# AdamYuan/Adypt

Measured on AMD Instinct MI355X. Metric: Mrays/sec (primary+secondary) Sponza 1920x1080 8-bounce; % HBM-read roofline, higher is better.
Workload: dtype f32; 1 GPU; sponza-like procedural stand-in (stand-in), 248964 triangles, 1920x1080, full wavefront path trace, maxBounce 8, tmpLifetime 16, 1 spp per step; one radiance gather per timed region; frames_in_flight=32, rays_warmup=62962782, comm=none, comm_ranks=0, devices=device 0, bounces_in_one_launch=True, rehearsal=False

## Files before the change

### adypt_amd/csrc/device/context.hpp

```cpp
#pragma once
#include "traverse.hpp"
#include "path.hpp"
#include "frame_plan.hpp"
#include "tunables.hpp"
#include "resources.hpp"
#include "../../../include/adypt_hip.h"

#include <string>
#include <vector>

using namespace adypt;

namespace {

constexpr int kMaxBounce = 32;
constexpr int kMaxFramesInFlight = 128;
constexpr int kRollMaxPixels = 1 << 22;
constexpr int kDefaultPipes = 1;

struct FrameCounters {
	uint32_t count[kMaxBounce + 1][kNumSegments * kCursorStride];
	uint32_t cursor[kMaxBounce + 1][kNumSegments * kCursorStride];
	uint32_t sh_count[kMaxBounce + 1][kNumSegments * kCursorStride];
	uint32_t sh_cursor[kMaxBounce + 1][kNumSegments * kCursorStride];
};

struct EventPair { Event a, b; int kind = 0; };

struct Pipe {
	Stream stream;
	Event done;
	FrameCounters *counters = nullptr;
	uint2 *spill = nullptr;
};

struct QueueWindow { size_t offset; uint32_t seg_cap; };

struct Queues {
	Buffer<float4> o[2], d[2], col[2], hit;
	Buffer<float4> done;
	Buffer<float4> sh_o, sh_d, sh_col, sh_hit;
	Buffer<RayStats> ray_stats;
};

}

struct adypt_ctx {
	int device = 0;
	std::string error;
	Tunables tun;

	static constexpr int kSobolSlots = 4;
	Pipe pipes[kMaxPipes];
	hipStream_t stream = nullptr;
	Event fork_ev;
// ... 101 lines not shown
```

### adypt_amd/csrc/device/frame_schedule.hpp

```cpp
#pragma once
#include "context.hpp"
#include "../../../include/adypt_host.h"

namespace {

struct PassArgs { SceneArgs sc; PixelArgs px; bool stats; };
PassArgs pass_args(const adypt_ctx *c)
{
	PassArgs a;
	fill_scene(c, &a.sc); fill_pixels(c, &a.px);
	a.stats = (c->instrumentation & 2) != 0;
	return a;
}

void launch_resolve(adypt_ctx *c, const FrameArgs &f, const PassArgs &a, int first, int count)
{
	const dim3 grid((c->n_local_px + 255) / 256), block(256);
	if(c->noise_stats) hipLaunchKernelGGL(k_resolve_noise, grid, block, 0, c->stream, f, a.sc, a.px, c->d_noise_moments.get(), first, count);
	else hipLaunchKernelGGL(k_resolve, grid, block, 0, c->stream, f, a.sc, a.px, first, count);
}

int resolve_batch_frames(adypt_ctx *c, int first, int count)
{
	if(count <= 0) return ADYPT_OK;
// ... 15 lines not shown
	return ADYPT_OK;
}

void drop_rolling(adypt_ctx *c)
{
	if(c->roll_frame[0] < 0 && c->roll_frame[1] < 0) return;
	(void)hipSetDevice(c->device);
	(void)hipStreamSynchronize(c->stream);
	for(int s = 0; s < 2; ++s) { (void)hipStreamSynchronize(c->pipes[1 + s].stream); c->roll_frame[s] = -1; }
}
inline void drop_lookahead(adypt_ctx *c) { c->ahead_count = 0; c->ahead_pos = 0; drop_rolling(c); }

int upload_sobol(adypt_ctx *c, int first, int m, float *dst)
{
	const int max_bounce = c->params.max_bounce;
	const int slot = c->sobol_next;
	c->sobol_next = (slot + 1) % adypt_ctx::kSobolSlots;
	HIP_TRY(c, hipEventSynchronize(c->sobol_done[slot]));
	std::vector<float> pts((size_t)m * 2 * max_bounce);
	int r = adypt_sobol_points(2 * max_bounce, first, m, pts.data());
	if(r != ADYPT_OK) return fail(c, r, adypt_host_last_error());
	float *padded = c->h_sobol[slot];
	memset(padded, 0, (size_t)m * 64 * sizeof(float));
	for(int k = 0; k < m; ++k) memcpy(&padded[(size_t)k * 64], &pts[(size_t)k * 2 * max_bounce], sizeof(float) * 2 * (size_t)max_bounce);
	HIP_TRY(c, hipMemcpyAsync(dst, padded, (size_t)m * 64 * sizeof(float), hipMemcpyHostToDevice, c->stream));
	HIP_TRY(c, hipEventRecord(c->sobol_done[slot], c->stream));
	return ADYPT_OK;
}

void launch_shade_first(adypt_ctx *c, hipStream_t stream, int k, const QueueWindow &win, const FrameArgs &f, const PassArgs &a)
{
	FrameCounters *ctr = c->pipes[k].counters;
	hipEvent_t stop = begin_timing(c, 1, stream);
	QueueArgs q = queue_args(c, win, 0, ctr->count[0], ctr->count[1], f.n_frames);
	audit_before(c, q, stream, k);
	hipLaunchKernelGGL(k_shade_first, dim3((unsigned)(c->n_local_px / kShadeThreads)), dim3(kShadeThreads), 0, stream, f, a.sc, q, a.px, a.stats ? 1 : 0);
	audit_after(c, q, stream, k);
	end_timing(stop, stream);
}

void roll_frame_args(const adypt_ctx *c, const PassPlan &p, int frame, int s, FrameArgs *f)
{
	fill_frame(c, f);
	f->spp = frame; f->n_frames = 1; f->frame_first = 0; f->frame_stride = 1; f->batched = 1;
	f->sun_query = p.sun_query;
	f->sobol = c->d_sobol + (size_t)s * 64;
	f->done = c->q.done + (size_t)s * (size_t)std::max(c->n_local_px, 64);
}

int roll_launch(adypt_ctx *c, const PassPlan &p, const PassArgs &a, int frame, int s)
{
	const Pipe &pipe = c->pipes[1 + s];
	const QueueWindow win = pipe_window(c, s, 2);
	FrameArgs f;
	roll_frame_args(c, p, frame, s, &f);
	int r = upload_sobol(c, frame, 1, c->d_sobol + (size_t)s * 64);
	if(r != ADYPT_OK) return r;
	if(frame % std::max(1, c->params.tmp_lifetime) == 0)
	{
		FrameArgs fc = f;
		fc.frame_stride = std::max(1, c->params.tmp_lifetime);
// ... 215 lines not shown
```

### adypt_amd/csrc/device/path.hpp

```cpp
#pragma once
#include "traverse.hpp"
#include "path_limits.hpp"

namespace adypt {

#ifndef ADYPT_PATH_SLOTS
#define ADYPT_PATH_SLOTS 352
#endif
constexpr int kPathSlots = ADYPT_PATH_SLOTS;
static_assert(kPathSlots >= kTraceThreads && kPathSlots <= 2 * kTraceThreads && kPathSlots % 32 == 0, "k_path: 256 <= slots <= 512");
constexpr int kTabFields = 10;
constexpr int kRareCap = 96;
static_assert(kRareCap >= 64 && kRareCap % 8 == 0 && kRareCap + 64 <= kTraceThreads, "k_path: the deferred ring holds a round's worth (rare_min <= 64), keeps PathCtl 16-byte aligned behind it, and leaves the to-shade ring a full batch when every path waits");
constexpr int kParkDwords = 8;
constexpr uint32_t kRingMiss = 0x8000u;
constexpr uint32_t kPwIdMask = (1u << kPwBounceShift) - 1u;
enum { T_PW = 0, T_DX, T_DY, T_DZ, T_CX, T_CY, T_CZ, T_OX, T_OY, T_OZ };

struct PathCtl {
	uint32_t n_shade, n_trace, live, busy;
	uint32_t h_shade, h_trace, rays, shaded;
	uint32_t lock, init_have, h_rare, pad[5];
};

// ... 276 lines not shown
					F3 dir = f3(0, 0, 1), color = f3(0, 0, 0), origin = f3(0, 0, 0), ret = f3(0, 0, 0), ret_in = f3(0, 0, 0);
					int32_t tri_idx = -1;
					float tu = 0.0f, tv = 0.0f;
					if(have)
					{
						pw = tab[T_PW * kPathSlots + sslot];
						dir = f3(__uint_as_float(tab[T_DX * kPathSlots + sslot]), __uint_as_float(tab[T_DY * kPathSlots + sslot]), __uint_as_float(tab[T_DZ * kPathSlots + sslot]));
						color = f3(__uint_as_float(tab[T_CX * kPathSlots + sslot]), __uint_as_float(tab[T_CY * kPathSlots + sslot]), __uint_as_float(tab[T_CZ * kPathSlots + sslot]));
						if(!miss) { tri_idx = (int32_t)tab[T_OX * kPathSlots + sslot]; tu = __uint_as_float(tab[T_OY * kPathSlots + sslot]); tv = __uint_as_float(tab[T_OZ * kPathSlots + sslot]); }
					}
					const int b = (int)((pw >> kPwBounceShift) & 31u);
					const int pi = (int)(pw & kPwIdMask);
					bool parked = (pw & kPathParked) != 0u;
					const bool last = b + 1 >= f.max_bounce;
					const bool query_back = SUN && (uint32_t)b == kPwShadow, query_next = SUN && f.sun_query != 0 && !query_back && have && tri_idx == -1;
					const int frame = (int)((uint32_t)pi / (uint32_t)f.n_local_px);
					const int L = pi - frame * f.n_local_px;
					TriCore tc;
#pragma unroll
					for(int i = 0; i < 20; ++i) asm volatile("" : "=v"(tc.v[i]));
					if(have && tri_idx != -1 && !query_back)
					{
						if(a.tri_remap) tri_idx = a.tri_remap[tri_idx];
						tc = load_tri_core(sc, tri_idx);
					}
					const bool sure = have && !query_next && (tri_idx == -1 || last);
					const uint32_t n_sure = (uint32_t)__popcll(__ballot(sure));
					const bool early = n_sure != 0u && !((seg_done >> home) & 1u);
					uint32_t rel;
					asm volatile("" : "=v"(rel));
					{
// ... 14 lines not shown
						sob_x = sp2.x; sob_y = sp2.y;
					}
					if(may_defer)
					{
						const bool rare = have && tri_idx != -1 && !last && __float_as_uint(tc.v[19]) != 0u;
						const unsigned long long rm = __ballot(rare);
						if(rm != 0ull && (uint32_t)__popcll(rm) <= a.defer_max)
						{
							const uint32_t room = (uint32_t)kRareCap - n_r, rr = lane_rank(rm);
							const bool defer = rare && rr < room;
							if(defer) to_rare[ring_r(h_r + n_r + rr)] = (uint16_t)sslot;
							n_r += min((uint32_t)__popcll(rm), room);
							have = have && !defer;
						}
					}

					bool alive = have, shaded = false, bad_mat = false;
					if(have)
					{
						if(parked) ret = f3(r4.x, r4.y, r4.z);
						ret_in = ret;
						if(query_next)
						{
							dir = f3(f.sun_query_dir[0], f.sun_query_dir[1], f.sun_query_dir[2]);
							origin = f3(__uint_as_float(tab[T_OX * kPathSlots + sslot]), __uint_as_float(tab[T_OY * kPathSlots + sslot]), __uint_as_float(tab[T_OZ * kPathSlots + sslot]));
						}
						else if(tri_idx == -1)
						{
							ret = fma3(color, f3(f.sun[0], f.sun[1], f.sun[2]), ret);
							alive = false;
						}
						else if(query_back) alive = false;
						else
						{
							const SurfaceInfo si = fetch_info(f, sc, tc, tri_idx, tu, tv);
							origin = si.origin;
							if(si.bad_mat) { alive = false; bad_mat = true; }
							else
							{
								shaded = true;
								const RngPoint rng{unorm8_to_float(shift16 & 0xffu), unorm8_to_float(shift16 >> 8), sob_x, sob_y};
								alive = respond(f, si, rng, b, dir, color, ret);
							}
						}
						if(!alive)
							f.done[pi] = make_float4(gl_min(ret.x, f.clamp), gl_min(ret.y, f.clamp), gl_min(ret.z, f.clamp), 1.0f);
					}
					wave_bad += (uint32_t)__popcll(__ballot(bad_mat));
					if(count_stats) wave_shaded += (uint32_t)__popcll(__ballot(shaded));
					if(alive)
					{
						if(__float_as_uint(ret.x) != __float_as_uint(ret_in.x) || __float_as_uint(ret.y) != __float_as_uint(ret_in.y) ||
						   __float_as_uint(ret.z) != __float_as_uint(ret_in.z))
						{
							f.done[pi] = make_float4(ret.x, ret.y, ret.z, 0.0f);
							parked = true;
// ... 120 lines not shown
```

### adypt_amd/csrc/device/scene_upload.hpp

```cpp
#pragma once
#include "context.hpp"
#include "../../../include/adypt_host.h"

#include <cstring>

namespace {

constexpr long kRefTrianglesAutoMaxMB = 1l << 20;

int upload_woop(adypt_ctx *c, const adypt_scene_desc *d)
{
	std::vector<float> woop;
	const float *wp = d->woop;
	if(!wp) { woop.resize((size_t)d->n_refs * 12); adypt_woop_matrices(d->triangles, d->tri_indices, d->n_refs, woop.data()); wp = woop.data(); }
	return upload(c, &c->d_woop, wp, (size_t)d->n_refs * 12);
}

int upload_triangles(adypt_ctx *c, const adypt_scene_desc *d)
{
	std::vector<float> packed((size_t)d->n_tris * kTriFloat4 * 4, 0.0f);
	const uint8_t *src = (const uint8_t *)d->triangles;
	for(int64_t i = 0; i < d->n_tris; ++i)
	{
		float *o = packed.data() + (size_t)i * kTriFloat4 * 4;
// ... 25 lines not shown
		if(matid < 0 || matid >= d->n_mats) continue;
		memcpy(&dtex, mat + (size_t)matid * 64, 4); memcpy(&illum, mat + (size_t)matid * 64 + 48, 4); memcpy(&shininess, mat + (size_t)matid * 64 + 52, 4);
		cls[(size_t)i] = (uint8_t)material_class(illum, shininess, d->n_textures != 0 && dtex >= 0 && dtex < d->n_textures);
	}
	return upload(c, &c->d_tri_class, cls.data(), cls.size());
}

int upload_textures_and_materials(adypt_ctx *c, const adypt_scene_desc *d)
{
	std::vector<uint32_t> texels;
	std::vector<int32_t> desc;
	for(int t = 0; t < d->n_textures; ++t)
	{
		const adypt_texture &tx = d->textures[t];
		if(tx.width <= 0 || tx.height <= 0 || !tx.rgb) return fail(c, ADYPT_E_INVALID, "adypt_create: bad texture " + std::to_string(t));
		desc.push_back((int32_t)texels.size()); desc.push_back(tx.width); desc.push_back(tx.height); desc.push_back(0);
		const size_t base = texels.size(), row = (size_t)tx.width + 1;
		if(base + row * (size_t)tx.height >= ((size_t)1 << 31)) return fail(c, ADYPT_E_INVALID, "adypt_create: more than 2^31 texels");
		texels.resize(base + row * (size_t)tx.height);
		for(int y = 0; y < tx.height; ++y)
		{
			uint32_t *o = texels.data() + base + row * (size_t)y;
			const uint8_t *in = tx.rgb + (size_t)y * tx.width * 3;
			for(int x = 0; x < tx.width; ++x) o[x] = (uint32_t)in[x * 3] | (uint32_t)in[x * 3 + 1] << 8 | (uint32_t)in[x * 3 + 2] << 16 | 0xff000000u;
			o[tx.width] = o[0];
		}
	}
	TRY_CREATE(upload(c, &c->d_texels, texels.data(), texels.size()));
	std::vector<uint8_t> mats((size_t)std::max<int64_t>(d->n_mats, 1) * kMatFloat4 * 16, 0);
	for(int64_t m = 0; m < d->n_mats; ++m)
	{
// ... 38 lines not shown
```

### adypt_amd/csrc/device/shade.hpp

```cpp
#pragma once
#include "canon_math.hpp"
#include "tile_layout.hpp"
#include "noise.hpp"

namespace adypt {

constexpr int kTraceThreads = 256;
constexpr int kLdsStackMax = 8;
constexpr int kNumSegments = 8;
constexpr int kCursorStride = 32;
constexpr int kShadeThreads = 256;
constexpr int kTriFloat4 = 8;
constexpr int kMatFloat4 = 5;
constexpr uint32_t kPathParked = 0x80000000u;
constexpr uint32_t kPathIdMask = 0x7fffffffu;
constexpr uint32_t kPathShadow = 0x40000000u;

struct DeviceStats {
	unsigned long long rays, nodes, tris, hits, shaded, overflows, bad_materials;
	uint32_t max_stack, pad;
	unsigned long long wave_profile[8];
	unsigned long long clock_cycles, clock_ticks;
	unsigned long long path_rays, path_nodes, path_tris, path_hits, path_shaded;
	unsigned long long audit_errors;
	uint32_t *host_overflow;
};
__device__ __forceinline__ void report_overflow(DeviceStats *st) { atomicAdd(&st->overflows, 1ull); *st->host_overflow = 1u; }

// ... 10 lines not shown
	uint32_t *cursor;
	uint2 *spill;
	DeviceStats *stats;
	uint32_t seg_cap;
	int32_t stack_size, lds_depth;
	uint32_t refill_min, chunk, bite, endgame;
	uint32_t packed;
	float tmin;
};

struct FrameArgs {
	float inv_proj[16], inv_view[16];
	float origin[3], tmin;
	float sun[3], clamp;
	const float *sobol;
	float4 *done;
	int32_t width, height;
	int32_t spp, subpixel, tmp_life, max_bounce;
	float sun_query_dir[3];
	int32_t sun_query;
	int32_t n_frames;
	int32_t frame_first, frame_stride;
	int32_t batched;
	int32_t n_local_px;
	int32_t blocks_x;
	int32_t rank, nranks;
	int32_t n_tris, n_mats, n_tex;
	int32_t deal_chunks;
};

struct SceneArgs {
	const float4 *triangles;
	const float4 *materials;
	const uint32_t *texels;
	const int32_t *local_blocks;
	const uint8_t *tri_class;
};

constexpr uint32_t kClassMiss = 0, kClassNone = 7;
// ... 167 lines not shown
	int x, y;
	if(L >= f.n_local_px || !local_pixel_xy(f, sc.local_blocks, L, &x, &y)) return;
	float4 acc = px.accum[L];
	NoiseMoments m = f.spp + first == 0 ? NoiseMoments{0.0f, 0.0f} : moments[L];
	for(int k = first; k < first + count; ++k)
	{
		const float4 r = f.done[(size_t)k * f.n_local_px + L];
		const float fs = (float)(f.spp + k), fs1 = (float)(f.spp + k + 1);
		acc = make_float4(fmaf(acc.x, fs, r.x) / fs1, fmaf(acc.y, fs, r.y) / fs1, fmaf(acc.z, fs, r.z) / fs1, 1.0f);
		m = noise_add_sample(m, f.spp + k, r.x, r.y, r.z);
	}
	px.accum[L] = acc;
	moments[L] = m;
}

__device__ __forceinline__ int pos_mod(int a, int n) { int r = a % n; return r < 0 ? r + n : r; }

struct __attribute__((packed, aligned(4))) TexelPair { uint32_t a, b; };
__device__ inline F3 sample_texture(const SceneArgs &sc, int4 d, float s, float t)
{
	const int w = d.y, h = d.z;
	const uint32_t *tx = sc.texels + d.x;
	const float uu = fmaf(s, (float)w, -0.5f), vv = fmaf(t, (float)h, -0.5f);
	float fu = floorf(uu), fv = floorf(vv);
	const float a = uu - fu, b = vv - fv;
	fu = gl_min(gl_max(fu, -1e9f), 1e9f); fv = gl_min(gl_max(fv, -1e9f), 1e9f);
	const int i0 = pos_mod((int)fu, w), j0 = pos_mod((int)fv, h);
	const int j1 = j0 + 1 == h ? 0 : j0 + 1;
	const TexelPair r0 = *(const TexelPair *)(tx + (size_t)j0 * (size_t)(w + 1) + i0), r1 = *(const TexelPair *)(tx + (size_t)j1 * (size_t)(w + 1) + i0);
	auto rgb = [](uint32_t p) { return f3(unorm8_to_float(p), unorm8_to_float(p >> 8), unorm8_to_float(p >> 16)); };
	const float w00 = (1.0f - a) * (1.0f - b), w10 = a * (1.0f - b), w01 = (1.0f - a) * b, w11 = a * b;
	F3 r = rgb(r0.a) * w00;
	r = fma3(rgb(r0.b), w10, r);
	r = fma3(rgb(r1.a), w01, r);
	r = fma3(rgb(r1.b), w11, r);
	return r;
}

struct TriCore { float v[20]; };
__device__ __forceinline__ TriCore load_tri_core(const SceneArgs &sc, int tri_idx)
{
	const float4 *p = sc.triangles + (size_t)tri_idx * kTriFloat4;
	const float4 a = p[0], b = p[1], c = p[2], d = p[3], e = p[4];
	TriCore t;
// ... 6 lines not shown
{
	F3 r = f3(a[0], a[1], a[2]) * u;
	r = fma3(f3(b[0], b[1], b[2]), v, r);
	r = fma3(f3(c[0], c[1], c[2]), w, r);
	return r;
}
__device__ __forceinline__ F3 textured_diffuse(const SceneArgs &sc, int tri_idx, int4 desc, float u, float v, float w)
{
	const float4 *p = sc.triangles + (size_t)tri_idx * kTriFloat4 + 5;
	const float4 a = p[0], b = p[1];
	const float ts = fmaf(b.x, w, fmaf(a.z, v, a.x * u));
	const float tt = fmaf(b.y, w, fmaf(a.w, v, a.y * u));
	return sample_texture(sc, desc, ts, tt);
}

struct Rng { float sx, sy; const float *sobol; };
__device__ __forceinline__ void sobol2(const Rng &r, int i, float *x, float *y)
{
	const float a = r.sobol[2 * i] + r.sx, b = r.sobol[2 * i + 1] + r.sy;
	*x = a - floorf(a); *y = b - floorf(b);
}
struct RngPoint { float sx, sy, qx, qy; };
__device__ __forceinline__ void sobol2(const RngPoint &r, int, float *x, float *y)
{
	const float a = r.qx + r.sx, b = r.qy + r.sy;
	*x = a - floorf(a); *y = b - floorf(b);
}
template <class RNG>
__device__ inline F3 sample_hemisphere(const RNG &rng, int b, float e)
{
	float rx, ry; sobol2(rng, b, &rx, &ry);
	rx *= 6.28318530718f;
	float sin_phi, cos_phi; canon_sincos(rx, &sin_phi, &cos_phi);
	const float cos_theta = canon_pow(1.0f - ry, 1.0f / (e + 1.0f));
	const float sin_theta = sqrtf(fmaf(-cos_theta, cos_theta, 1.0f));
	return normalize3(f3(sin_theta * cos_phi, sin_theta * sin_phi, cos_theta));
}
__device__ inline F3 align_direction(F3 dir, F3 target)
{
	const F3 a = fabsf(target.x) > 0.01f ? f3(0, 1, 0) : f3(1, 0, 0);
	const F3 u = normalize3(cross3(a, target));
	const F3 v = cross3(target, u);
	F3 r = u * dir.x;
	r = fma3(v, dir.y, r);
	r = fma3(target, dir.z, r);
	return r;
}

__device__ __forceinline__ void finish_path(const FrameArgs &f, const PixelArgs &px, int pi, int L, F3 ret)
{
	const F3 r = f3(gl_min(ret.x, f.clamp), gl_min(ret.y, f.clamp), gl_min(ret.z, f.clamp));
// ... 1 lines not shown
	const float4 old = px.accum[L];
	const float fs = (float)f.spp, fs1 = (float)(f.spp + 1);
	px.accum[L] = make_float4(fmaf(old.x, fs, r.x) / fs1, fmaf(old.y, fs, r.y) / fs1, fmaf(old.z, fs, r.z) / fs1, 1.0f);
}

struct SurfaceInfo { F3 origin, normal, diffuse, specular, emission; int illum0; float shininess, ior; bool bad_mat; };
__device__ __forceinline__ SurfaceInfo fetch_info(const FrameArgs &f, const SceneArgs &sc, const TriCore &tc, int tri_idx, float tu, float tv)
{
	SurfaceInfo s;
	const float *tri = tc.v;
	const int matid = __float_as_int(tri[18]);
	const float w = 1.0f - tu - tv;
	s.normal = normalize3(bary3(tri + 9, tri + 12, tri + 15, tu, tv, w));
	s.origin = bary3(tri + 0, tri + 3, tri + 6, tu, tv, w);
	s.bad_mat = matid < 0 || matid >= f.n_mats;
	s.diffuse = s.specular = s.emission = f3(0, 0, 0); s.illum0 = 0; s.shininess = 0.0f; s.ior = 1.0f;
	if(!s.bad_mat)
	{
		const float4 *mp = sc.materials + (size_t)matid * kMatFloat4;
		const float4 md = mp[0], me = mp[1], ms = mp[2], mx = mp[3], mt = mp[4];
		const int dtex = __float_as_int(md.x);
		s.illum0 = __float_as_int(mx.x); s.shininess = mx.y; s.ior = mx.w;
		const int4 tex_desc = make_int4(__float_as_int(mt.x), __float_as_int(mt.y), __float_as_int(mt.z), 0);
		if(f.n_tex != 0 && dtex != -1 && dtex >= 0 && dtex < f.n_tex) s.diffuse = textured_diffuse(sc, tri_idx, tex_desc, tu, tv, w);
		else s.diffuse = f3(md.y, md.z, md.w);
		s.specular = f3(ms.y, ms.z, ms.w);
		s.emission = f3(me.y, me.z, me.w);
	}
	return s;
}

__device__ __forceinline__ SurfaceInfo fetch_info(const FrameArgs &f, const SceneArgs &sc, int tri_idx, float tu, float tv)
{
	return fetch_info(f, sc, load_tri_core(sc, tri_idx), tri_idx, tu, tv);
}

template <class RNG>
__device__ __forceinline__ bool respond(const FrameArgs &f, const SurfaceInfo &si, const RNG &rng, int b, F3 &dir, F3 &color, F3 &ret)
// ... 74 lines not shown
	uint32_t local = chunk * kShadeThreads + threadIdx.x;
	if(sc.tri_class)
	{
		uint32_t key = kClassNone;
		if(local < n_in)
		{
			const int tri = __float_as_int(q.hit[3 * ((size_t)seg * q.seg_cap + local)]);
			key = tri < 0 || tri >= f.n_tris ? kClassMiss : (uint32_t)sc.tri_class[tri];
		}
		local = chunk * kShadeThreads + bin_by_key(key);
	}
	const uint32_t slot_in = seg * q.seg_cap + local;
	bool alive = local < n_in;
	F3 origin = f3(0, 0, 0), dir = f3(0, 0, 1), color = f3(0, 0, 0), ret = f3(0, 0, 0);
	int L = 0, pi = 0;
	const float *sobol = f.sobol;
	bool shaded = false, bad_mat = false, parked = false, escaped = false;
	F3 ret_in = f3(0, 0, 0);
	if(alive)
	{
		const float4 rd = q.ray_d[slot_in];
		const F3 h = ld3(q.hit, slot_in);
		color = ld3(q.col, slot_in);
		dir = f3(rd.x, rd.y, rd.z);
		pi = (int)(__float_as_uint(rd.w) & kPathIdMask);
		L = pi;
		if(f.batched)
		{
			const int frame = (int)((uint32_t)pi / (uint32_t)f.n_local_px);
			L = pi - frame * f.n_local_px;
			sobol += frame * 64;
		}
		parked = (__float_as_uint(rd.w) & kPathParked) != 0u;
		if(parked) { const float4 r4 = f.done[pi]; ret = f3(r4.x, r4.y, r4.z); }
		ret_in = ret;
		const int tri_idx = __float_as_int(h.x);
		const float tu = h.y, tv = h.z;
		if(store_cache) px.cache[L] = make_float4(h.x, tu, tv, 0.0f);

		if(tri_idx == -1)
		{
			if(sh.enabled) escaped = true;
			else ret = fma3(color, f3(f.sun[0], f.sun[1], f.sun[2]), ret);
			alive = false;
		}
		else
		{
			const SurfaceInfo si = fetch_info(f, sc, tri_idx, tu, tv);
			origin = si.origin;
			if(si.bad_mat) { alive = false; bad_mat = true; }
			else
			{
				shaded = true;
				const uint8_t *sh = px.shift + (size_t)L * 2;
				const Rng rng{unorm8_to_float(sh[0]), unorm8_to_float(sh[1]), sobol};
				alive = respond(f, si, rng, b, dir, color, ret);
			}
		}
		if(!alive && !escaped) finish_path(f, px, pi, L, ret);
	}
	{
		const unsigned long long mb = __ballot(bad_mat);
		if(mb && (threadIdx.x & 63) == 0) atomicAdd(&px.stats->bad_materials, (unsigned long long)__popcll(mb));
		if(count_stats)
		{
			const int n_shaded = __syncthreads_count(shaded);
			if(n_shaded && threadIdx.x == 0) atomicAdd(&px.stats->shaded, (unsigned long long)n_shaded);
		}
	}
	const uint32_t slot = append_slot(alive, q.count_out + seg * kCursorStride, seg * q.seg_cap);
// ... 23 lines not shown
}

__global__ __launch_bounds__(kShadeThreads, 7) void k_shade(FrameArgs f, SceneArgs sc, QueueArgs q, PixelArgs px, ShadowArgs sh, int b, int store_cache, int count_stats)
{
	const uint32_t seg = blockIdx.x & (kNumSegments - 1), chunk = blockIdx.x >> 3;
	const uint32_t n_in = q.count_in[seg * kCursorStride];
	if(chunk * kShadeThreads >= n_in) return;
	shade_chunk(f, sc, q, px, sh, b, store_cache, count_stats, seg, chunk, n_in);
}

__global__ __launch_bounds__(kShadeThreads, 6) void k_shade_first(FrameArgs f, SceneArgs sc, QueueArgs q, PixelArgs px, int count_stats)
{
	const uint32_t L = blockIdx.x * kShadeThreads + threadIdx.x;
	int x = 0, y = 0;
	const bool valid = L < (uint32_t)f.n_local_px && local_pixel_xy(f, sc.local_blocks, (int)L, &x, &y);
	Rng rng{0.0f, 0.0f, f.sobol};
	if(valid)
	{
		const uint8_t *sh = px.shift + (size_t)L * 2;
		rng.sx = unorm8_to_float(sh[0]); rng.sy = unorm8_to_float(sh[1]);
	}
	SurfaceInfo si;
	si.origin = si.normal = si.diffuse = si.specular = si.emission = f3(0, 0, 0); si.illum0 = 0; si.shininess = 0.0f; si.ior = 1.0f; si.bad_mat = false;
	F3 cam_dir = f3(0, 0, 1);
	bool hit = false;
	int group_now = -1;
	unsigned long long n_shaded = 0, n_bad = 0;
	for(int ordinal = 0; ordinal < f.n_frames; ++ordinal)
	{
		const int frame = f.frame_first + ordinal * f.frame_stride;
		const int group = frame_group(f, frame);
		if(group != group_now)
		{
			group_now = group;
			if(valid)
			{
// ... 5 lines not shown
				hit = tri_idx != -1;
				if(hit) si = fetch_info(f, sc, tri_idx, h.y, h.z);
			}
		}
		const int pi = frame * f.n_local_px + (int)L;
		bool alive = valid, query = false;
		F3 dir = cam_dir, color = f3(1.0f, 1.0f, 1.0f), ret = f3(0, 0, 0);
		if(valid)
		{
			if(!hit && f.sun_query) { query = true; dir = f3(f.sun_query_dir[0], f.sun_query_dir[1], f.sun_query_dir[2]); }
			else if(!hit) { ret = fma3(color, f3(f.sun[0], f.sun[1], f.sun[2]), ret); alive = false; }
			else if(si.bad_mat) { alive = false; ++n_bad; }
			else
			{
				++n_shaded;
				Rng r = rng; r.sobol = f.sobol + frame * 64;
				alive = respond(f, si, r, 0, dir, color, ret);
			}
			if(!alive) finish_path(f, px, pi, (int)L, ret);
		}
		const uint32_t seg = ((uint32_t)ordinal * gridDim.x + blockIdx.x) & (kNumSegments - 1);
		const uint32_t slot = append_slot(alive, q.count_out + seg * kCursorStride, seg * q.seg_cap);
		if(alive)
		{
			if(query) st3(q.out_o, slot, f.origin[0], f.origin[1], f.origin[2]);
			else st3(q.out_o, slot, si.origin.x, si.origin.y, si.origin.z);
			bool parked = false;
			if(__float_as_uint(ret.x) != 0u || __float_as_uint(ret.y) != 0u || __float_as_uint(ret.z) != 0u)
			{
				f.done[pi] = make_float4(ret.x, ret.y, ret.z, 0.0f);
				parked = true;
			}
// ... 37 lines not shown
__device__ __forceinline__ F3 viewer_color(const FrameArgs &f, const SceneArgs &sc, DeviceStats *stats, int tri_idx, float u, float v, int viewer_type)
{
	F3 color = f3(0, 0, 0);
	if(tri_idx == -1) return color;
	const int matid = __float_as_int(sc.triangles[(size_t)tri_idx * kTriFloat4 + 4].z);
	if(matid < 0 || matid >= f.n_mats) { atomicAdd(&stats->bad_materials, 1ull); return color; }
	const float4 *mp = sc.materials + (size_t)matid * kMatFloat4;
	const float w = 1.0f - u - v;
	if(viewer_type == 0)
	{
		const float4 md = mp[0];
		const int dtex = __float_as_int(md.x);
		if(f.n_tex != 0 && dtex != -1 && dtex >= 0 && dtex < f.n_tex)
		{
			const float4 mt = mp[4];
			color = textured_diffuse(sc, tri_idx, make_int4(__float_as_int(mt.x), __float_as_int(mt.y), __float_as_int(mt.z), 0), u, v, w);
		}
		else color = f3(md.y, md.z, md.w);
	}
	else if(viewer_type == 1) { const float4 ms = mp[2]; color = f3(ms.y, ms.z, ms.w); }
	else if(viewer_type == 2) { const float4 me = mp[1]; color = f3(me.y, me.z, me.w); }
	else if(viewer_type == 4 || viewer_type == 5)
	{
		const TriCore tc = load_tri_core(sc, tri_idx);
		const float *tri = tc.v;
		color = viewer_type == 4 ? normalize3(bary3(tri + 9, tri + 12, tri + 15, u, v, w)) : bary3(tri + 0, tri + 3, tri + 6, u, v, w);
	}
	return color;
}

__device__ __forceinline__ uint32_t unorm8(float c)
// ... 73 lines not shown
```

### adypt_amd/csrc/device/tracer.hip

```cpp
#include "context.hpp"
#include "ctx_access.hpp"
#include "../../../include/adypt_hip.h"
#include "../../../include/adypt_host.h"

#include <algorithm>
#include <atomic>
#include <cstdio>
#include <cstdlib>
#include <cstring>
#include <string>
#include <type_traits>
#include <vector>

using namespace adypt;

namespace {

thread_local std::string g_create_error;

__global__ void k_clear_counters(uint4 *p, uint32_t n16) { const uint32_t i = blockIdx.x * blockDim.x + threadIdx.x; if(i < n16) p[i] = make_uint4(0, 0, 0, 0); }

constexpr uint32_t kAuditPoison = 0xffffffffu;
__global__ void k_audit_poison(float4 *out_d, size_t n, uint32_t *seen, size_t n_seen)
{
// ... 234 lines not shown
	HIP_TRY(c, hipGetLastError());
	return ADYPT_OK;
}

void fill_frame(const adypt_ctx *c, FrameArgs *f)
{
	memset(f, 0, sizeof(*f));
	memcpy(f->inv_proj, c->inv_proj, 64); memcpy(f->inv_view, c->inv_view, 64);
	memcpy(f->origin, c->origin, 12);
	f->tmin = c->params.ray_tmin;
	memcpy(f->sun, c->params.sun, 12);
	f->clamp = c->params.clamp;
	f->width = c->width; f->height = c->height;
	f->spp = c->spp; f->subpixel = c->params.subpixel; f->tmp_life = c->params.tmp_lifetime; f->max_bounce = c->params.max_bounce;
	f->sobol = c->d_sobol; f->done = c->q.done; f->n_frames = 1; f->frame_first = 0; f->frame_stride = 1; f->batched = 0;
	f->n_local_px = c->n_local_px; f->blocks_x = c->blocks_x; f->rank = c->rank; f->nranks = c->nranks;
	f->n_tris = (int32_t)c->n_tris; f->n_mats = (int32_t)c->n_mats; f->n_tex = c->n_tex;
	f->deal_chunks = c->deal_chunks;
	memcpy(f->sun_query_dir, c->sun_dir, 12); f->sun_query = 0;
}
void fill_scene(const adypt_ctx *c, SceneArgs *s)
{
	s->triangles = (const float4 *)c->d_triangles;
	s->materials = (const float4 *)c->d_materials;
	s->texels = (const uint32_t *)c->d_texels;
	s->local_blocks = (const int32_t *)c->d_local_blocks;
	s->tri_class = (const uint8_t *)c->d_tri_class;
}
void fill_pixels(const adypt_ctx *c, PixelArgs *p)
{
	p->accum = c->d_accum; p->cache = c->d_cache; p->cache_next = c->d_cache_next; p->shift = c->d_shift; p->stats = c->d_stats;
// ... 63 lines not shown
int load_shift(adypt_ctx *c)
{
	if(c->shift_loaded && c->shift_seed_loaded == c->params.shift_seed) return ADYPT_OK;
	std::vector<uint8_t> full((size_t)c->width * c->height * 2), local((size_t)c->n_local_px * 2, 0);
	adypt_shift_bytes(c->params.shift_seed, c->width, c->height, full.data());
	for_each_local_pixel(c->local_blocks, c->width, c->height, [&](size_t L, int x, int y) {
		local[L * 2] = full[((size_t)y * c->width + x) * 2];
		local[L * 2 + 1] = full[((size_t)y * c->width + x) * 2 + 1];
	});
	HIP_TRY(c, hipStreamSynchronize(c->stream));
	if(!local.empty()) HIP_TRY(c, hipMemcpy(c->d_shift, local.data(), local.size(), hipMemcpyHostToDevice));
	c->shift_loaded = true; c->shift_seed_loaded = c->params.shift_seed;
	return ADYPT_OK;
}

int alloc_queues_raw(adypt_ctx *c, int fif)
{
	c->q = Queues{};
	const size_t npx = (size_t)std::max(c->n_local_px, 64);
	const size_t paths = npx * (size_t)fif;
	if(paths >= ((size_t)1 << 31)) return fail(c, ADYPT_E_INVALID, "frames in flight x pixels exceeds 2^31 paths");
	c->seg_cap = seg_slots_for(c, fif);
	c->capacity = (int64_t)c->seg_cap * kNumSegments;
	c->frames_in_flight = fif;
	size_t nq = (size_t)c->capacity;
	for(int n = 2; n <= kMaxPipes; ++n)
		nq = std::max(nq, (size_t)n * kNumSegments * (size_t)seg_slots_for(c, (fif + n - 1) / n));
	c->alloc_slots = nq;
	for(int i = 0; i < 2; ++i)
	{
		HIP_TRY(c, c->q.o[i].alloc(nq * sizeof(float4)));
		HIP_TRY(c, c->q.d[i].alloc(nq * sizeof(float4)));
		HIP_TRY(c, c->q.col[i].alloc(nq * sizeof(float4)));
	}
	HIP_TRY(c, c->q.hit.alloc(nq * sizeof(float4)));
	HIP_TRY(c, c->q.done.alloc(npx * (size_t)std::max(fif, 2) * sizeof(float4)));
	return ADYPT_OK;
}

int alloc_queues(adypt_ctx *c, int fif)
{
	const int previous = c->queues_ok ? c->frames_in_flight : 0;
	int r = alloc_queues_raw(c, fif);
	c->queues_ok = r == ADYPT_OK;
	if(r == ADYPT_OK) return r;
	const std::string why = c->error;
	(void)hipGetLastError();
	if(previous > 0 && previous != fif && alloc_queues_raw(c, previous) == ADYPT_OK)
	{
		c->queues_ok = true;
		c->error = why + " (kept " + std::to_string(previous) + " frames in flight)";
// ... 832 lines not shown
```

### adypt_amd/csrc/measure/k_path_blocks.py

```python
import sys
d = sys.argv[1]
import os
COUNT = os.environ.get("ADYPT_BLOCKS_COUNT", "0") != "0"
SET = os.environ.get("ADYPT_BLOCKS_SET", "trip")
SETS = {"trip": ["setup", "exchange", "shade", "trip", "A_pop", "A_choose", "A_push", "B_tri_load", "B_node_load", "C_woop", "D_slab", "E_flush"],
        "shade": ["shade", "S_parked", "S_miss", "S_surface", "S_textured", "S_glossy", "S_diffuse", "S_mirror", "S_dielectric", "S_dead", "S_alive", "S_replace"],
        "rare": ["trip", "shade", "A_pop_spill", "A_push_spill", "div_slow", "S_fetch_more", "S_early", "X_lock_spin", "exchange", "setup", "F_try", "S_defer"]}
LANES = os.environ.get("ADYPT_BLOCKS_LANES", "0") != "0"
SETS_LANES = {"trip": ["trip", "A_choose", "C_woop", "D_slab", "E_flush"], "shade": ["S_surface", "S_textured", "S_glossy", "S_diffuse", "S_dielectric"],
              "rare": ["S_miss", "S_mirror", "S_dead", "S_alive", "S_replace"],
              "wait": ["W_idle", "W_wait", "W_two", "W_three", "W_four"]}
NAMES = SETS_LANES[SET] if LANES else SETS[SET]


def edit(name, pairs):
    p = d + "/" + name
    s = open(p).read()
    for old, new in pairs:
        assert s.count(old) == 1, (name, s.count(old), old[:70])
        s = s.replace(old, new)
    open(p, "w").write(s)


def enter(n):
# ... 50 lines not shown
    ("						if(parked) r4 = f.done[pi];", "						if(parked) { " + enter("S_parked") + " r4 = f.done[pi]; " + leave("S_parked") + " }"),
    ("							ret = fma3(color, f3(f.sun[0], f.sun[1], f.sun[2]), ret); // pathtracer.glsl:130-135 (a query that came back empty: the sun is visible)\n							alive = false;",
     "							" + enter("S_miss") + "\n							ret = fma3(color, f3(f.sun[0], f.sun[1], f.sun[2]), ret); // pathtracer.glsl:130-135 (a query that came back empty: the sun is visible)\n							alive = false;\n							" + leave("S_miss")),
    ("							const SurfaceInfo si = fetch_info(f, sc, tc, tri_idx, tu, tv);", "							" + enter("S_surface") + "\n							const SurfaceInfo si = fetch_info(f, sc, tc, tri_idx, tu, tv);"),
    ("						if(rm != 0ull && (uint32_t)__popcll(rm) <= a.defer_max)\n						{", "						if(rm != 0ull && (uint32_t)__popcll(rm) <= a.defer_max)\n						{\n							" + enter("S_defer")),
    ("							have = have && !defer;\n						}", "							have = have && !defer;\n							" + leave("S_defer") + "\n						}"),
    ("								alive = respond(f, si, rng, b, dir, color, ret);\n							}\n						}", "								alive = respond(f, si, rng, b, dir, color, ret);\n							}\n							" + leave("S_surface") + "\n						}"),
    ("						if(!alive) // main()'s clamp (pathtracer.glsl:224); the running mean is k_resolve's, in frame order (a k_path pass is always batched)\n							f.done[pi] = make_float4(gl_min(ret.x, f.clamp), gl_min(ret.y, f.clamp), gl_min(ret.z, f.clamp), 1.0f);",
     "						if(!alive) { " + enter("S_dead") + "\n							f.done[pi] = make_float4(gl_min(ret.x, f.clamp), gl_min(ret.y, f.clamp), gl_min(ret.z, f.clamp), 1.0f); " + leave("S_dead") + " }"),
    ("					if(alive)\n					{\n						if(__float_as_uint(ret.x) != __float_as_uint(ret_in.x)", "					if(alive)\n					{\n						" + enter("S_alive") + "\n						if(__float_as_uint(ret.x) != __float_as_uint(ret_in.x)"),
    ("						tab[T_OX * kPathSlots + sslot] = __float_as_uint(origin.x); tab[T_OY * kPathSlots + sslot] = __float_as_uint(origin.y); tab[T_OZ * kPathSlots + sslot] = __float_as_uint(origin.z);\n					}\n					// ---------------- paths that ended",
     "						tab[T_OX * kPathSlots + sslot] = __float_as_uint(origin.x); tab[T_OY * kPathSlots + sslot] = __float_as_uint(origin.y); tab[T_OZ * kPathSlots + sslot] = __float_as_uint(origin.z);\n						" + leave("S_alive") + "\n					}\n					// ---------------- paths that ended"),
    ("					if(repl) load_path(a, idx, sslot);", "					if(repl) { " + enter("S_replace") + " load_path(a, idx, sslot); " + leave("S_replace") + " }"),
]
SHADE_HPP = [
    ("		if(f.n_tex != 0 && dtex != -1 && dtex >= 0 && dtex < f.n_tex) s.diffuse = textured_diffuse(sc, tri_idx, tex_desc, tu, tv, w);\n		else s.diffuse = f3(md.y, md.z, md.w);\n		s.specular = f3(ms.y, ms.z, ms.w);",
     "		if(f.n_tex != 0 && dtex != -1 && dtex >= 0 && dtex < f.n_tex) { " + enter("S_textured") + " s.diffuse = textured_diffuse(sc, tri_idx, tex_desc, tu, tv, w); " + leave("S_textured") + " }\n		else s.diffuse = f3(md.y, md.z, md.w);\n		s.specular = f3(ms.y, ms.z, ms.w);"),
    ("		if(e > 0.3f)\n		{\n			const F3 r = reflect3(dir, normal), shv = sample_hemisphere(rng, b, e);", "		if(e > 0.3f)\n		{\n			" + enter("S_glossy") + "\n			const F3 r = reflect3(dir, normal), shv = sample_hemisphere(rng, b, e);"),
    ("			done = true;\n		}\n		else illum = 1;", "			done = true;\n			" + leave("S_glossy") + "\n		}\n		else illum = 1;"),
    ("		if(illum == 1)\n		{\n			dir = align_direction(sample_hemisphere(rng, b, 0.0f), normal);\n			color = color * diffuse;\n		}",
     "		if(illum == 1)\n		{\n			" + enter("S_diffuse") + "\n			dir = align_direction(sample_hemisphere(rng, b, 0.0f), normal);\n			color = color * diffuse;\n			" + leave("S_diffuse") + "\n		}"),
    ("		else if(illum >= 3 && illum <= 5)\n		{\n			color = color * specular;\n			dir = reflect3(dir, normal);\n		}",
     "		else if(illum >= 3 && illum <= 5)\n		{\n			" + enter("S_mirror") + "\n			color = color * specular;\n			dir = reflect3(dir, normal);\n			" + leave("S_mirror") + "\n		}"),
    ("		else if(illum == 6 || illum == 7)\n		{\n			float eta = ior;", "		else if(illum == 6 || illum == 7)\n		{\n			" + enter("S_dielectric") + "\n			float eta = ior;"),
    ("			else dir = reflect3(dir, normal);\n		}\n	}\n	return alive;", "			else dir = reflect3(dir, normal);\n			" + leave("S_dielectric") + "\n		}\n	}\n	return alive;"),
]
edit("shade.hpp", SHADE_HPP)
pairs = SHADE_PATH + [
    ("						if(early && lane == 0) rel = atomicAdd(&a.cursor[cur], n_sure);", "						if(early && lane == 0) { " + enter("S_early") + " rel = atomicAdd(&a.cursor[cur], n_sure); " + leave("S_early") + " }"),
    ("						while(served < n_dead) // (wave-uniform) the rest: paths that ended unexpectedly, or the home segment has run out\n						{", "						while(served < n_dead) // (wave-uniform) the rest: paths that ended unexpectedly, or the home segment has run out\n						{\n							" + enter("S_fetch_more")),
# ... 24 lines not shown
```

Before: 8383 Mrays/s.

## Precompute hemisphere sample tables, pow2 texture wrap, and magic-number path-id division

```diff
diff --git a/adypt_amd/csrc/device/context.hpp b/adypt_amd/csrc/device/context.hpp
--- a/adypt_amd/csrc/device/context.hpp
+++ b/adypt_amd/csrc/device/context.hpp
@@ -14,6 +14,7 @@
 namespace {
 
 constexpr int kMaxBounce = 32;
+static_assert(kMaxBounce == kSampleTabBounces, "the sampling tables have a row per bounce");
 constexpr int kMaxFramesInFlight = 128;
 constexpr int kRollMaxPixels = 1 << 22;
 constexpr int kDefaultPipes = 1;
@@ -39,6 +40,7 @@
 struct Queues {
 	Buffer<float4> o[2], d[2], col[2], hit;
 	Buffer<float4> done;
+	Buffer<float2> phi_tab, theta_tab;
 	Buffer<float4> sh_o, sh_d, sh_col, sh_hit;
 	Buffer<RayStats> ray_stats;
 };
diff --git a/adypt_amd/csrc/device/frame_schedule.hpp b/adypt_amd/csrc/device/frame_schedule.hpp
--- a/adypt_amd/csrc/device/frame_schedule.hpp
+++ b/adypt_amd/csrc/device/frame_schedule.hpp
@@ -53,6 +53,8 @@
 int upload_sobol(adypt_ctx *c, int first, int m, float *dst)
 {
 	const int max_bounce = c->params.max_bounce;
+	const size_t row0 = (size_t)(dst - c->d_sobol.get()) / 64;
+	if((row0 + (size_t)m) * kSampleTabBounces * 256 * sizeof(float2) > c->q.phi_tab.bytes()) return fail(c, ADYPT_E_STATE, "upload_sobol: more frames than the sampling tables hold");
 	const int slot = c->sobol_next;
 	c->sobol_next = (slot + 1) % adypt_ctx::kSobolSlots;
 	HIP_TRY(c, hipEventSynchronize(c->sobol_done[slot]));
@@ -64,6 +66,9 @@
 	for(int k = 0; k < m; ++k) memcpy(&padded[(size_t)k * 64], &pts[(size_t)k * 2 * max_bounce], sizeof(float) * 2 * (size_t)max_bounce);
 	HIP_TRY(c, hipMemcpyAsync(dst, padded, (size_t)m * 64 * sizeof(float), hipMemcpyHostToDevice, c->stream));
 	HIP_TRY(c, hipEventRecord(c->sobol_done[slot], c->stream));
+	hipLaunchKernelGGL(k_sample_tables, dim3((unsigned)max_bounce, (unsigned)m), dim3(256), 0, c->stream, (const float *)dst,
+	                   c->q.phi_tab + row0 * kSampleTabBounces * 256, c->q.theta_tab + row0 * kSampleTabBounces * 256);
+	HIP_TRY(c, hipGetLastError());
 	return ADYPT_OK;
 }
 
@@ -84,6 +89,7 @@
 	f->spp = frame; f->n_frames = 1; f->frame_first = 0; f->frame_stride = 1; f->batched = 1;
 	f->sun_query = p.sun_query;
 	f->sobol = c->d_sobol + (size_t)s * 64;
+	f->phi_tab = c->q.phi_tab + (size_t)s * kSampleTabBounces * 256; f->theta_tab = c->q.theta_tab + (size_t)s * kSampleTabBounces * 256;
 	f->done = c->q.done + (size_t)s * (size_t)std::max(c->n_local_px, 64);
 }
 
diff --git a/adypt_amd/csrc/device/path.hpp b/adypt_amd/csrc/device/path.hpp
--- a/adypt_amd/csrc/device/path.hpp
+++ b/adypt_amd/csrc/device/path.hpp
@@ -314,7 +314,7 @@
 					bool parked = (pw & kPathParked) != 0u;
 					const bool last = b + 1 >= f.max_bounce;
 					const bool query_back = SUN && (uint32_t)b == kPwShadow, query_next = SUN && f.sun_query != 0 && !query_back && have && tri_idx == -1;
-					const int frame = (int)((uint32_t)pi / (uint32_t)f.n_local_px);
+					const int frame = (int)path_id_div((uint32_t)pi, f.px_div);
 					const int L = pi - frame * f.n_local_px;
 					TriCore tc;
 #pragma unroll
@@ -359,6 +359,13 @@
 							have = have && !defer;
 						}
 					}
+					float2 ph, th;
+					asm volatile("" : "=v"(ph.x), "=v"(ph.y), "=v"(th.x), "=v"(th.y));
+					if(have)
+					{
+						const uint32_t row = (uint32_t)(frame * kSampleTabBounces + b) * 256u;
+						ph = f.phi_tab[row + (shift16 & 0xffu)]; th = f.theta_tab[row + (shift16 >> 8)];
+					}
 
 					bool alive = have, shaded = false, bad_mat = false;
 					if(have)
@@ -384,7 +391,7 @@
 							else
 							{
 								shaded = true;
-								const RngPoint rng{unorm8_to_float(shift16 & 0xffu), unorm8_to_float(shift16 >> 8), sob_x, sob_y};
+								const RngPoint rng{shift16, sob_x, sob_y, ph, th};
 								alive = respond(f, si, rng, b, dir, color, ret);
 							}
 						}
diff --git a/adypt_amd/csrc/device/path_id_div.hpp b/adypt_amd/csrc/device/path_id_div.hpp
--- /dev/null
+++ b/adypt_amd/csrc/device/path_id_div.hpp
@@ -0,0 +1,34 @@
+#pragma once
+#include <cstdint>
+#include "path_limits.hpp"
+
+#ifndef ADYPT_HOST_DEVICE
+#ifdef __HIPCC__
+#define ADYPT_HOST_DEVICE __host__ __device__ __forceinline__
+#else
+#define ADYPT_HOST_DEVICE inline
+#endif
+#endif
+
+namespace adypt {
+
+struct PathIdDiv { uint32_t mul, shift; };
+
+inline PathIdDiv path_id_div_of(uint32_t d)
+{
+	uint32_t l = 0;
+	while(((uint64_t)1 << l) < d) ++l;
+	const uint64_t p = (uint64_t)1 << (kPwBounceShift + l);
+	return PathIdDiv{(uint32_t)((p + d - 1) / d), l};
+}
+
+ADYPT_HOST_DEVICE uint32_t path_id_div(uint32_t n, PathIdDiv d)
+{
+#ifdef __HIP_DEVICE_COMPILE__
+	return __umulhi(n << (32u - kPwBounceShift), d.mul) >> d.shift;
+#else
+	return (uint32_t)(((uint64_t)(n << (32u - kPwBounceShift)) * d.mul) >> 32) >> d.shift;
+#endif
+}
+
+}
diff --git a/adypt_amd/csrc/device/scene_upload.hpp b/adypt_amd/csrc/device/scene_upload.hpp
--- a/adypt_amd/csrc/device/scene_upload.hpp
+++ b/adypt_amd/csrc/device/scene_upload.hpp
@@ -63,7 +63,8 @@
 	{
 		const adypt_texture &tx = d->textures[t];
 		if(tx.width <= 0 || tx.height <= 0 || !tx.rgb) return fail(c, ADYPT_E_INVALID, "adypt_create: bad texture " + std::to_string(t));
-		desc.push_back((int32_t)texels.size()); desc.push_back(tx.width); desc.push_back(tx.height); desc.push_back(0);
+		desc.push_back((int32_t)texels.size()); desc.push_back(tx.width); desc.push_back(tx.height);
+		desc.push_back(is_pow2(tx.width) && is_pow2(tx.height) ? 1 : 0);
 		const size_t base = texels.size(), row = (size_t)tx.width + 1;
 		if(base + row * (size_t)tx.height >= ((size_t)1 << 31)) return fail(c, ADYPT_E_INVALID, "adypt_create: more than 2^31 texels");
 		texels.resize(base + row * (size_t)tx.height);
diff --git a/adypt_amd/csrc/device/shade.hpp b/adypt_amd/csrc/device/shade.hpp
--- a/adypt_amd/csrc/device/shade.hpp
+++ b/adypt_amd/csrc/device/shade.hpp
@@ -2,6 +2,8 @@
 #include "canon_math.hpp"
 #include "tile_layout.hpp"
 #include "noise.hpp"
+#include "path_id_div.hpp"
+#include "texture_wrap.hpp"
 
 namespace adypt {
 
@@ -12,6 +14,7 @@
 constexpr int kShadeThreads = 256;
 constexpr int kTriFloat4 = 8;
 constexpr int kMatFloat4 = 5;
+constexpr int kSampleTabBounces = 32;
 constexpr uint32_t kPathParked = 0x80000000u;
 constexpr uint32_t kPathIdMask = 0x7fffffffu;
 constexpr uint32_t kPathShadow = 0x40000000u;
@@ -52,6 +55,7 @@
 	float origin[3], tmin;
 	float sun[3], clamp;
 	const float *sobol;
+	const float2 *phi_tab, *theta_tab;
 	float4 *done;
 	int32_t width, height;
 	int32_t spp, subpixel, tmp_life, max_bounce;
@@ -61,6 +65,7 @@
 	int32_t frame_first, frame_stride;
 	int32_t batched;
 	int32_t n_local_px;
+	PathIdDiv px_div;
 	int32_t blocks_x;
 	int32_t rank, nranks;
 	int32_t n_tris, n_mats, n_tex;
@@ -258,8 +263,6 @@
 	moments[L] = m;
 }
 
-__device__ __forceinline__ int pos_mod(int a, int n) { int r = a % n; return r < 0 ? r + n : r; }
-
 struct __attribute__((packed, aligned(4))) TexelPair { uint32_t a, b; };
 __device__ inline F3 sample_texture(const SceneArgs &sc, int4 d, float s, float t)
 {
@@ -269,9 +272,11 @@
 	float fu = floorf(uu), fv = floorf(vv);
 	const float a = uu - fu, b = vv - fv;
 	fu = gl_min(gl_max(fu, -1e9f), 1e9f); fv = gl_min(gl_max(fv, -1e9f), 1e9f);
-	const int i0 = pos_mod((int)fu, w), j0 = pos_mod((int)fv, h);
+	int i0, j0;
+	if(__ballot(d.w == 0) == 0ull) { i0 = pos_mod_pow2((int)fu, w); j0 = pos_mod_pow2((int)fv, h); }
+	else { i0 = pos_mod((int)fu, w); j0 = pos_mod((int)fv, h); }
 	const int j1 = j0 + 1 == h ? 0 : j0 + 1;
-	const TexelPair r0 = *(const TexelPair *)(tx + (size_t)j0 * (size_t)(w + 1) + i0), r1 = *(const TexelPair *)(tx + (size_t)j1 * (size_t)(w + 1) + i0);
+	const TexelPair r0 = *(const TexelPair *)(tx + (uint32_t)(j0 * (w + 1) + i0)), r1 = *(const TexelPair *)(tx + (uint32_t)(j1 * (w + 1) + i0));
 	auto rgb = [](uint32_t p) { return f3(unorm8_to_float(p), unorm8_to_float(p >> 8), unorm8_to_float(p >> 16)); };
 	const float w00 = (1.0f - a) * (1.0f - b), w10 = a * (1.0f - b), w01 = (1.0f - a) * b, w11 = a * b;
 	F3 r = rgb(r0.a) * w00;
@@ -308,27 +313,50 @@
 	return sample_texture(sc, desc, ts, tt);
 }
 
-struct Rng { float sx, sy; const float *sobol; };
-__device__ __forceinline__ void sobol2(const Rng &r, int i, float *x, float *y)
-{
-	const float a = r.sobol[2 * i] + r.sx, b = r.sobol[2 * i + 1] + r.sy;
-	*x = a - floorf(a); *y = b - floorf(b);
-}
-struct RngPoint { float sx, sy, qx, qy; };
-__device__ __forceinline__ void sobol2(const RngPoint &r, int, float *x, float *y)
-{
-	const float a = r.qx + r.sx, b = r.qy + r.sy;
-	*x = a - floorf(a); *y = b - floorf(b);
-}
+__device__ __forceinline__ float shifted(float q, uint32_t byte) { const float a = q + unorm8_to_float(byte); return a - floorf(a); }
+__device__ __forceinline__ float2 lobe_phi(float rx)
+{
+	rx *= 6.28318530718f;
+	float sin_phi, cos_phi; canon_sincos(rx, &sin_phi, &cos_phi);
+	return make_float2(sin_phi, cos_phi);
+}
+__device__ __forceinline__ float2 lobe_theta(float ry, float e)
+{
+	const float cos_theta = canon_pow(1.0f - ry, 1.0f / (e + 1.0f));
+	return make_float2(cos_theta, sqrtf(fmaf(-cos_theta, cos_theta, 1.0f)));
+}
+__global__ __launch_bounds__(256) void k_sample_tables(const float *sobol, float2 *phi_tab, float2 *theta_tab)
+{
+	const uint32_t b = blockIdx.x, frame = blockIdx.y, at = (frame * kSampleTabBounces + b) * 256u + threadIdx.x;
+	const float2 q = *(const float2 *)(sobol + frame * 64 + 2 * b);
+	phi_tab[at] = lobe_phi(shifted(q.x, threadIdx.x));
+	theta_tab[at] = lobe_theta(shifted(q.y, threadIdx.x), 0.0f);
+}
+
+struct Rng { uint32_t shift16; const float *sobol; const float2 *phi, *theta; };
+__device__ __forceinline__ Rng frame_rng(const FrameArgs &f, int frame, uint32_t shift16)
+{
+	return Rng{shift16, f.sobol + frame * 64, f.phi_tab + (size_t)frame * (kSampleTabBounces * 256), f.theta_tab + (size_t)frame * (kSampleTabBounces * 256)};
+}
+__device__ __forceinline__ void sobol2(const Rng &r, int i, float *x, float *y) { *x = shifted(r.sobol[2 * i], r.shift16 & 0xffu); *y = shifted(r.sobol[2 * i + 1], r.shift16 >> 8); }
+__device__ __forceinline__ float2 table_phi(const Rng &r, int i) { return r.phi[i * 256 + (int)(r.shift16 & 0xffu)]; }
+__device__ __forceinline__ float2 table_theta(const Rng &r, int i) { return r.theta[i * 256 + (int)(r.shift16 >> 8)]; }
+struct RngPoint { uint32_t shift16; float qx, qy; float2 phi, theta; };
+__device__ __forceinline__ void sobol2(const RngPoint &r, int, float *x, float *y) { *x = shifted(r.qx, r.shift16 & 0xffu); *y = shifted(r.qy, r.shift16 >> 8); }
+__device__ __forceinline__ float2 table_phi(const RngPoint &r, int) { return r.phi; }
+__device__ __forceinline__ float2 table_theta(const RngPoint &r, int) { return r.theta; }
 template <class RNG>
 __device__ inline F3 sample_hemisphere(const RNG &rng, int b, float e)
 {
-	float rx, ry; sobol2(rng, b, &rx, &ry);
-	rx *= 6.28318530718f;
-	float sin_phi, cos_phi; canon_sincos(rx, &sin_phi, &cos_phi);
-	const float cos_theta = canon_pow(1.0f - ry, 1.0f / (e + 1.0f));
-	const float sin_theta = sqrtf(fmaf(-cos_theta, cos_theta, 1.0f));
-	return normalize3(f3(sin_theta * cos_phi, sin_theta * sin_phi, cos_theta));
+	const float2 ph = table_phi(rng, b);
+	float2 th;
+	if(e == 0.0f) th = table_theta(rng, b);
+	else
+	{
+		float rx, ry; sobol2(rng, b, &rx, &ry);
+		th = lobe_theta(ry, e);
+	}
+	return normalize3(f3(th.y * ph.y, th.y * ph.x, th.x));
 }
 __device__ inline F3 align_direction(F3 dir, F3 target)
 {
@@ -360,14 +388,15 @@
 	s.normal = normalize3(bary3(tri + 9, tri + 12, tri + 15, tu, tv, w));
 	s.origin = bary3(tri + 0, tri + 3, tri + 6, tu, tv, w);
 	s.bad_mat = matid < 0 || matid >= f.n_mats;
-	s.diffuse = s.specular = s.emission = f3(0, 0, 0); s.illum0 = 0; s.shininess = 0.0f; s.ior = 1.0f;
+	asm volatile("" : "=v"(s.diffuse.x), "=v"(s.diffuse.y), "=v"(s.diffuse.z), "=v"(s.specular.x), "=v"(s.specular.y), "=v"(s.specular.z));
+	asm volatile("" : "=v"(s.emission.x), "=v"(s.emission.y), "=v"(s.emission.z), "=v"(s.illum0), "=v"(s.shininess), "=v"(s.ior));
 	if(!s.bad_mat)
 	{
 		const float4 *mp = sc.materials + (size_t)matid * kMatFloat4;
 		const float4 md = mp[0], me = mp[1], ms = mp[2], mx = mp[3], mt = mp[4];
 		const int dtex = __float_as_int(md.x);
 		s.illum0 = __float_as_int(mx.x); s.shininess = mx.y; s.ior = mx.w;
-		const int4 tex_desc = make_int4(__float_as_int(mt.x), __float_as_int(mt.y), __float_as_int(mt.z), 0);
+		const int4 tex_desc = make_int4(__float_as_int(mt.x), __float_as_int(mt.y), __float_as_int(mt.z), __float_as_int(mt.w));
 		if(f.n_tex != 0 && dtex != -1 && dtex >= 0 && dtex < f.n_tex) s.diffuse = textured_diffuse(sc, tri_idx, tex_desc, tu, tv, w);
 		else s.diffuse = f3(md.y, md.z, md.w);
 		s.specular = f3(ms.y, ms.z, ms.w);
@@ -472,7 +501,7 @@
 	bool alive = local < n_in;
 	F3 origin = f3(0, 0, 0), dir = f3(0, 0, 1), color = f3(0, 0, 0), ret = f3(0, 0, 0);
 	int L = 0, pi = 0;
-	const float *sobol = f.sobol;
+	int frame = 0;
 	bool shaded = false, bad_mat = false, parked = false, escaped = false;
 	F3 ret_in = f3(0, 0, 0);
 	if(alive)
@@ -485,9 +514,8 @@
 		L = pi;
 		if(f.batched)
 		{
-			const int frame = (int)((uint32_t)pi / (uint32_t)f.n_local_px);
+			frame = (int)((uint32_t)pi / (uint32_t)f.n_local_px);
 			L = pi - frame * f.n_local_px;
-			sobol += frame * 64;
 		}
 		parked = (__float_as_uint(rd.w) & kPathParked) != 0u;
 		if(parked) { const float4 r4 = f.done[pi]; ret = f3(r4.x, r4.y, r4.z); }
@@ -510,8 +538,7 @@
 			else
 			{
 				shaded = true;
-				const uint8_t *sh = px.shift + (size_t)L * 2;
-				const Rng rng{unorm8_to_float(sh[0]), unorm8_to_float(sh[1]), sobol};
+				const Rng rng = frame_rng(f, frame, *(const uint16_t *)(px.shift + (size_t)L * 2));
 				alive = respond(f, si, rng, b, dir, color, ret);
 			}
 		}
@@ -565,12 +592,7 @@
 	const uint32_t L = blockIdx.x * kShadeThreads + threadIdx.x;
 	int x = 0, y = 0;
 	const bool valid = L < (uint32_t)f.n_local_px && local_pixel_xy(f, sc.local_blocks, (int)L, &x, &y);
-	Rng rng{0.0f, 0.0f, f.sobol};
-	if(valid)
-	{
-		const uint8_t *sh = px.shift + (size_t)L * 2;
-		rng.sx = unorm8_to_float(sh[0]); rng.sy = unorm8_to_float(sh[1]);
-	}
+	const uint32_t shift16 = valid ? *(const uint16_t *)(px.shift + (size_t)L * 2) : 0u;
 	SurfaceInfo si;
 	si.origin = si.normal = si.diffuse = si.specular = si.emission = f3(0, 0, 0); si.illum0 = 0; si.shininess = 0.0f; si.ior = 1.0f; si.bad_mat = false;
 	F3 cam_dir = f3(0, 0, 1);
@@ -606,8 +628,7 @@
 			else
 			{
 				++n_shaded;
-				Rng r = rng; r.sobol = f.sobol + frame * 64;
-				alive = respond(f, si, r, 0, dir, color, ret);
+				alive = respond(f, si, frame_rng(f, frame, shift16), 0, dir, color, ret);
 			}
 			if(!alive) finish_path(f, px, pi, (int)L, ret);
 		}
@@ -675,7 +696,7 @@
 		if(f.n_tex != 0 && dtex != -1 && dtex >= 0 && dtex < f.n_tex)
 		{
 			const float4 mt = mp[4];
-			color = textured_diffuse(sc, tri_idx, make_int4(__float_as_int(mt.x), __float_as_int(mt.y), __float_as_int(mt.z), 0), u, v, w);
+			color = textured_diffuse(sc, tri_idx, make_int4(__float_as_int(mt.x), __float_as_int(mt.y), __float_as_int(mt.z), __float_as_int(mt.w)), u, v, w);
 		}
 		else color = f3(md.y, md.z, md.w);
 	}
diff --git a/adypt_amd/csrc/device/texture_wrap.hpp b/adypt_amd/csrc/device/texture_wrap.hpp
--- /dev/null
+++ b/adypt_amd/csrc/device/texture_wrap.hpp
@@ -0,0 +1,17 @@
+#pragma once
+
+#ifndef ADYPT_HOST_DEVICE
+#ifdef __HIPCC__
+#define ADYPT_HOST_DEVICE __host__ __device__ __forceinline__
+#else
+#define ADYPT_HOST_DEVICE inline
+#endif
+#endif
+
+namespace adypt {
+
+ADYPT_HOST_DEVICE int pos_mod(int a, int n) { int r = a % n; return r < 0 ? r + n : r; }
+ADYPT_HOST_DEVICE int pos_mod_pow2(int a, int n) { return a & (n - 1); }
+ADYPT_HOST_DEVICE bool is_pow2(int n) { return n > 0 && (n & (n - 1)) == 0; }
+
+}
diff --git a/adypt_amd/csrc/device/tracer.hip b/adypt_amd/csrc/device/tracer.hip
--- a/adypt_amd/csrc/device/tracer.hip
+++ b/adypt_amd/csrc/device/tracer.hip
@@ -272,7 +272,9 @@
 	f->width = c->width; f->height = c->height;
 	f->spp = c->spp; f->subpixel = c->params.subpixel; f->tmp_life = c->params.tmp_lifetime; f->max_bounce = c->params.max_bounce;
 	f->sobol = c->d_sobol; f->done = c->q.done; f->n_frames = 1; f->frame_first = 0; f->frame_stride = 1; f->batched = 0;
+	f->phi_tab = c->q.phi_tab; f->theta_tab = c->q.theta_tab;
 	f->n_local_px = c->n_local_px; f->blocks_x = c->blocks_x; f->rank = c->rank; f->nranks = c->nranks;
+	f->px_div = path_id_div_of((uint32_t)std::max(c->n_local_px, 1));
 	f->n_tris = (int32_t)c->n_tris; f->n_mats = (int32_t)c->n_mats; f->n_tex = c->n_tex;
 	f->deal_chunks = c->deal_chunks;
 	memcpy(f->sun_query_dir, c->sun_dir, 12); f->sun_query = 0;
@@ -366,6 +368,7 @@
 	return ADYPT_OK;
 }
 
+inline size_t sample_tab_entries(int frames) { return (size_t)std::max(frames, 2) * kSampleTabBounces * 256; }
 int alloc_queues_raw(adypt_ctx *c, int fif)
 {
 	c->q = Queues{};
@@ -387,6 +390,8 @@
 	}
 	HIP_TRY(c, c->q.hit.alloc(nq * sizeof(float4)));
 	HIP_TRY(c, c->q.done.alloc(npx * (size_t)std::max(fif, 2) * sizeof(float4)));
+	HIP_TRY(c, c->q.phi_tab.alloc(sample_tab_entries(fif) * sizeof(float2)));
+	HIP_TRY(c, c->q.theta_tab.alloc(sample_tab_entries(fif) * sizeof(float2)));
 	return ADYPT_OK;
 }
 
diff --git a/adypt_amd/csrc/measure/k_path_blocks.py b/adypt_amd/csrc/measure/k_path_blocks.py
--- a/adypt_amd/csrc/measure/k_path_blocks.py
+++ b/adypt_amd/csrc/measure/k_path_blocks.py
@@ -5,7 +5,7 @@
 SET = os.environ.get("ADYPT_BLOCKS_SET", "trip")
 SETS = {"trip": ["setup", "exchange", "shade", "trip", "A_pop", "A_choose", "A_push", "B_tri_load", "B_node_load", "C_woop", "D_slab", "E_flush"],
         "shade": ["shade", "S_parked", "S_miss", "S_surface", "S_textured", "S_glossy", "S_diffuse", "S_mirror", "S_dielectric", "S_dead", "S_alive", "S_replace"],
-        "rare": ["trip", "shade", "A_pop_spill", "A_push_spill", "div_slow", "S_fetch_more", "S_early", "X_lock_spin", "exchange", "setup", "F_try", "S_defer"]}
+        "rare": ["trip", "shade", "A_pop_spill", "A_push_spill", "div_slow", "S_fetch_more", "S_early", "X_lock_spin", "exchange", "S_wrap_mod", "F_try", "S_defer"]}
 LANES = os.environ.get("ADYPT_BLOCKS_LANES", "0") != "0"
 SETS_LANES = {"trip": ["trip", "A_choose", "C_woop", "D_slab", "E_flush"], "shade": ["S_surface", "S_textured", "S_glossy", "S_diffuse", "S_dielectric"],
               "rare": ["S_miss", "S_mirror", "S_dead", "S_alive", "S_replace"],
@@ -88,6 +88,7 @@
     ("					if(repl) load_path(a, idx, sslot);", "					if(repl) { " + enter("S_replace") + " load_path(a, idx, sslot); " + leave("S_replace") + " }"),
 ]
 SHADE_HPP = [
+    ("	else { i0 = pos_mod((int)fu, w); j0 = pos_mod((int)fv, h); }", "	else { " + enter("S_wrap_mod") + " i0 = pos_mod((int)fu, w); j0 = pos_mod((int)fv, h); " + leave("S_wrap_mod") + " }"),
     ("		if(f.n_tex != 0 && dtex != -1 && dtex >= 0 && dtex < f.n_tex) s.diffuse = textured_diffuse(sc, tri_idx, tex_desc, tu, tv, w);\n		else s.diffuse = f3(md.y, md.z, md.w);\n		s.specular = f3(ms.y, ms.z, ms.w);",
      "		if(f.n_tex != 0 && dtex != -1 && dtex >= 0 && dtex < f.n_tex) { " + enter("S_textured") + " s.diffuse = textured_diffuse(sc, tri_idx, tex_desc, tu, tv, w); " + leave("S_textured") + " }\n		else s.diffuse = f3(md.y, md.z, md.w);\n		s.specular = f3(ms.y, ms.z, ms.w);"),
     ("		if(e > 0.3f)\n		{\n			const F3 r = reflect3(dir, normal), shv = sample_hemisphere(rng, b, e);", "		if(e > 0.3f)\n		{\n			" + enter("S_glossy") + "\n			const F3 r = reflect3(dir, normal), shv = sample_hemisphere(rng, b, e);"),
```

Result: slower. 8144 Mrays/s (-2.9%).
